# ostrosco/comms-rs

Hardware: NVIDIA B200
Metric: FIR/FFT Msamples/s (higher is better)
Workload: dtype f32

## Files before the change

comms-rs_b200/csrc/fir_tc_kernel.cu:

```cuda
#include <cuda_fp16.h>

#include <vector>

#include "fir_kernels.cuh"

namespace cb {

namespace tc {

constexpr int ROWS = 128;
constexpr int RS = 32;
constexpr int TILE = ROWS * RS;
constexpr int NCW = 6;
constexpr int NCONV = 32 * NCW;
constexpr int W_EPI = 2 * NCW;
constexpr int W_MMA = W_EPI + 4, W_TMA = W_EPI + 5;
constexpr int NTHREADS = 32 * (W_TMA + 1);
static_assert(W_EPI % 4 == 0, "epilogue warp w must own TMEM sub-partition w % 4");
constexpr int A_PART = 18432;
constexpr int A_STAGE = 2 * A_PART;
constexpr int OUT_PITCH = 272;
constexpr int OUT_WARP = 32 * OUT_PITCH;

struct Args {
    const float2 *x;
    const float2 *halo;
    float2 *y;
    const float2 *hist_in;
    float2 *hist_out;
    const uint4 *bimg;
    unsigned long long n;
    unsigned hist_len;
    float tap_inv_scale;
    unsigned *fix_count;
    unsigned *fix_list;
    const uint32_t *x16;
    uint32_t *y16;
    float in_scale, out_scale;
};

__device__ __forceinline__ int quant_i16(float v, float scale)
{
    const int q = __float2int_rz(__fmul_rn(scale, v));
    return min(max(q, -32768), 32767);
}
__device__ __forceinline__ uint32_t pack_i16(int lo, int hi) { return __byte_perm((uint32_t)lo, (uint32_t)hi, 0x5410); }
__device__ __forceinline__ float2 widen_iq16(uint32_t w, float scale)
{
    return make_float2(__fmul_rn(scale, (float)(int16_t)(w & 0xFFFFu)), __fmul_rn(scale, (float)(int16_t)(w >> 16)));
}

__device__ __forceinline__ void mbar_arrive(uint64_t *bar)
{
    asm volatile("mbarrier.arrive.shared::cta.b64 _, [%0];" ::"r"(smem_u32(bar)) : "memory");
}
__device__ __forceinline__ void tc_fence_before() { asm volatile("tcgen05.fence::before_thread_sync;" ::: "memory"); }
__device__ __forceinline__ void tc_fence_after() { asm volatile("tcgen05.fence::after_thread_sync;" ::: "memory"); }
__device__ __forceinline__ void tc_commit(uint64_t *bar)
{
    asm volatile("tcgen05.commit.cta_group::1.mbarrier::arrive::one.shared::cluster.b64 [%0];" ::"r"(smem_u32(bar))
                 : "memory");
}
__device__ __forceinline__ bool elect_one()
{
    uint32_t pred;
    asm volatile(
        "{\n"
        ".reg .pred P;\n"
        "elect.sync _|P, 0xffffffff;\n"
        "selp.u32 %0, 1, 0, P;\n"
        "}\n"
        : "=r"(pred));
    return pred != 0;
}
__device__ __forceinline__ void tc_mma(uint32_t tmem_d, uint64_t adesc, uint64_t bdesc, uint32_t idesc, uint32_t accumulate)
{
    asm volatile(
        "{\n"
        ".reg .pred p;\n"
        "setp.ne.b32 p, %4, 0;\n"
        "tcgen05.mma.cta_group::1.kind::f16 [%0], %1, %2, %3, p;\n"
        "}\n" ::"r"(tmem_d),
        "l"(adesc), "l"(bdesc), "r"(idesc), "r"(accumulate)
        : "memory");
}
__device__ __forceinline__ void tc_ld32(uint32_t taddr, uint32_t *r)
{
    asm volatile(
        "tcgen05.ld.sync.aligned.32x32b.x32.b32 "
        "{%0, %1, %2, %3, %4, %5, %6, %7, %8, %9, %10, %11, %12, %13, %14, %15, "
        "%16, %17, %18, %19, %20, %21, %22, %23, %24, %25, %26, %27, %28, %29, %30, %31}, [%32];\n"
        : "=r"(r[0]), "=r"(r[1]), "=r"(r[2]), "=r"(r[3]), "=r"(r[4]), "=r"(r[5]), "=r"(r[6]), "=r"(r[7]), "=r"(r[8]),
          "=r"(r[9]), "=r"(r[10]), "=r"(r[11]), "=r"(r[12]), "=r"(r[13]), "=r"(r[14]), "=r"(r[15]), "=r"(r[16]),
          "=r"(r[17]), "=r"(r[18]), "=r"(r[19]), "=r"(r[20]), "=r"(r[21]), "=r"(r[22]), "=r"(r[23]), "=r"(r[24]),
          "=r"(r[25]), "=r"(r[26]), "=r"(r[27]), "=r"(r[28]), "=r"(r[29]), "=r"(r[30]), "=r"(r[31])
        : "r"(taddr));
}
__device__ __forceinline__ void tc_wait_ld() { asm volatile("tcgen05.wait::ld.sync.aligned;" ::: "memory"); }

__device__ __forceinline__ uint64_t tc_desc(uint32_t saddr)
{
    uint64_t d = (uint64_t)((saddr >> 4) & 0x3FFF);
    d |= (uint64_t)1 << 16;
    d |= (uint64_t)(1024 >> 4) << 32;
    d |= (uint64_t)1 << 46;
    d |= (uint64_t)2 << 61;
    return d;
}

__device__ __forceinline__ uint32_t swz128(uint32_t o) { return o ^ (((o >> 7) & 7) << 4); }

__device__ __noinline__ float4 iq16_edge_pair(const Args &a, long long g, int halo);

#ifdef CB_FTC_STATS
__device__ unsigned long long *g_ftc_dbg = nullptr;
#define FTC_DECL unsigned long long st_[8] = {0}; long long t_ = clock64()
#define FTC_T(cond, k)                               \
    if (cond) {                                      \
        const long long now_ = clock64();            \
        st_[k] += (unsigned long long)(now_ - t_);   \
        t_ = now_;                                   \
    }
#define FTC_OUT(cond, role)                                                                            \
    if ((cond) && g_ftc_dbg != nullptr)                                                                \
        for (int k_ = 0; k_ < 8; ++k_) g_ftc_dbg[((size_t)blockIdx.x * 5 + (role)) * 8 + k_] = st_[k_]
#else
#define FTC_DECL
#define FTC_T(cond, k)
#define FTC_OUT(cond, role)
#endif

template <int KB, int NRAW, bool IQ16 = false, bool SMIN = false>
__global__ void __launch_bounds__(NTHREADS, 1) fir_tc_kernel(const __grid_constant__ Args a)
{
    constexpr int HALO = RS * (KB - 1);
    constexpr int NPAIR = (TILE + HALO) / 2;
    constexpr int NLD = (NPAIR + NCONV - 1) / NCONV;
    constexpr int B_BYTES = KB * 16384;
    constexpr uint32_t IDESC128 = (1u << 4) | ((128u >> 3) << 17) | ((128u >> 4) << 24);
    constexpr uint32_t IDESC64 = (1u << 4) | ((64u >> 3) << 17) | ((128u >> 4) << 24);

    extern __shared__ __align__(1024) unsigned char smem_raw[];
    unsigned char *smem = smem_raw + ((1024u - (smem_u32(smem_raw) & 1023u)) & 1023u);
    unsigned char *sB = smem;
    unsigned char *sA = smem + B_BYTES;
    unsigned char *sOut = sA + 2 * A_STAGE;
    constexpr int RAWB = (TILE + HALO) * (IQ16 ? 4 : 8);
    unsigned char *sRaw = sOut + 4 * OUT_WARP;
    __shared__ __align__(8) uint64_t raw_full[NRAW], raw_empty[NRAW];
    __shared__ __align__(8) uint64_t a_full[2], a_empty[2], t_full[2], t_empty[2], sc_ready[8];
    __shared__ uint32_t tmem_slot;
    __shared__ float red_max[2][2][NCW];
    __shared__ uint32_t red_min[2][2][NCW];
    __shared__ unsigned fix_seen[2];
    __shared__ float inv_scale[8];

    const int tid = threadIdx.x, warp = tid >> 5, lane = tid & 31;
    const unsigned long long ntiles = (a.n + TILE - 1) / TILE;

    if (tid == 0) {
        fix_seen[0] = fix_seen[1] = 0u;
        for (int i = 0; i < 2; ++i) {
            mbar_init(&a_full[i], NCONV);
            mbar_init(&a_empty[i], 1);
            mbar_init(&t_full[i], 1);
            mbar_init(&t_empty[i], 128);
        }
        for (int i = 0; i < 8; ++i) mbar_init(&sc_ready[i], 1);
        for (int i = 0; i < NRAW; ++i) {
            mbar_init(&raw_full[i], 1);
            mbar_init(&raw_empty[i], NCONV);
        }
        fence_mbar_init();
    }
    if (warp == W_MMA) {
        asm volatile("tcgen05.alloc.cta_group::1.sync.aligned.shared::cta.b32 [%0], %1;" ::"r"(smem_u32(&tmem_slot)),
                     "r"(256)
                     : "memory");
        asm volatile("tcgen05.relinquish_alloc_permit.cta_group::1.sync.aligned;" ::: "memory");
    }
    for (int i = tid; i < B_BYTES / 16; i += NTHREADS) reinterpret_cast<uint4 *>(sB)[i] = a.bimg[i];
    for (int i = tid; i < NRAW * RAWB / 16; i += NTHREADS) reinterpret_cast<uint4 *>(sRaw)[i] = make_uint4(0u, 0u, 0u, 0u);
    fence_proxy_async();
    tc_fence_before();
    __syncthreads();
    tc_fence_after();
    const uint32_t tmem_base = tmem_slot;

    if (warp == W_TMA) {
        unsigned long long it = 0;
        FTC_DECL;
        for (unsigned long long tile = blockIdx.x; tile < ntiles; tile += gridDim.x, ++it) {
            const int rs = (int)(it % NRAW);
            const uint32_t ph = (uint32_t)((it / NRAW) & 1);
            const long long g0 = (long long)tile * TILE - HALO;
            const long long g_lo = g0 < 0 ? 0 : g0;
            long long g_hi = g0 + TILE + HALO;
            if (g_hi > (long long)a.n) g_hi = (long long)a.n & (IQ16 ? ~3ll : ~1ll);
            if (g_hi < g_lo) g_hi = g_lo;
            FTC_T(lane == 0, 0);
            mbar_wait_long(&raw_empty[rs], ph ^ 1);
            FTC_T(lane == 0, 1);
            unsigned char *dstb = sRaw + rs * RAWB;
            if constexpr (IQ16) {
                if (lane == 0) mbar_arrive_expect_tx(&raw_full[rs], (uint32_t)((g_hi - g_lo) * 4));
                __syncwarp();
                for (long long g = g_lo + (long long)lane * 512; g < g_hi; g += 32 * 512) {
                    const long long n = g_hi - g < 512 ? g_hi - g : 512;
                    tma_load_1d(dstb + (g - g0) * 4, a.x16 + g, (uint32_t)(n * 4), &raw_full[rs]);
                }
                continue;
            }
            if (lane == 0) mbar_arrive_expect_tx(&raw_full[rs], (uint32_t)((g_hi - g_lo) * 8 + (g0 < 0 ? -g0 * 8 : 0)));
            __syncwarp();
            if (g0 < 0 && lane == 31) tma_load_1d(dstb, a.halo + (HALO + g0), (uint32_t)(-g0 * 8), &raw_full[rs]);
            for (long long g = g_lo + (long long)lane * 256; g < g_hi; g += 32 * 256) {
                const long long n = g_hi - g < 256 ? g_hi - g : 256;
                tma_load_1d(dstb + (g - g0) * 8, a.x + g, (uint32_t)(n * 8), &raw_full[rs]);
            }
        }
        FTC_OUT(lane == 0, 0);
    } else if (warp < W_EPI) {
        const int grp = warp / NCW, gt = tid - grp * NCONV, gw = warp - grp * NCW;
        if (a.hist_out != nullptr && blockIdx.x == 0 && grp == 0) {
            const long long H = a.hist_len;
            for (long long i = gt; i < H; i += NCONV) {
                const long long g = (long long)a.n - H + i;
                if constexpr (IQ16) a.hist_out[i] = g >= 0 ? widen_iq16(a.x16[g], a.in_scale) : a.hist_in[H + g];
                else a.hist_out[i] = g >= 0 ? a.x[g] : a.hist_in[H + g];
            }
        }
        unsigned long long it = grp;
        FTC_DECL;
        for (unsigned long long tile = blockIdx.x + (unsigned long long)grp * gridDim.x; tile < ntiles;
             tile += 2ull * gridDim.x, it += 2) {
            const int s = grp;
            const uint32_t ph = (uint32_t)((it >> 1) & 1);
            const long long t0 = (long long)tile * TILE;
            float4 raw[NLD];
            float mx = 0.f;
            uint32_t mnu = 0xffffffffu;
            const int rs = (int)(it % NRAW);
            FTC_T(gt == 0, 0);
            mbar_wait(&raw_full[rs], (uint32_t)((it / NRAW) & 1));
            FTC_T(gt == 0, 1);
            const float4 *rawt = reinterpret_cast<const float4 *>(sRaw + rs * RAWB);
            if constexpr (IQ16) {
                uint2 rw[NLD];
#pragma unroll
                for (int i = 0; i < NLD; ++i) {
                    const int q = gt + i * NCONV;
                    rw[i] = q < NPAIR ? reinterpret_cast<const uint2 *>(rawt)[q] : make_uint2(0u, 0u);
                }
#pragma unroll
                for (int i = 0; i < NLD; ++i) {
                    const float2 s0 = widen_iq16(rw[i].x, a.in_scale), s1 = widen_iq16(rw[i].y, a.in_scale);
                    raw[i] = make_float4(s0.x, s0.y, s1.x, s1.y);
                }
                if (t0 < HALO || t0 + TILE > ((long long)a.n & ~3ll)) {
#pragma unroll
                    for (int i = 0; i < NLD; ++i) {
                        const int q = gt + i * NCONV;
                        const long long g = t0 - HALO + 2 * q;
                        if (q < NPAIR && (g < 0 || g + 1 >= ((long long)a.n & ~3ll))) raw[i] = iq16_edge_pair(a, g, HALO);
                    }
                    if (t0 < HALO) {
#pragma unroll
                        for (int i = 0; i < NLD; ++i) {
                            const float4 v = raw[i];
                            mnu = min(mnu, quiet_key<SMIN>(v, fmaxf(fmaxf(fabsf(v.x), fabsf(v.y)), fmaxf(fabsf(v.z), fabsf(v.w)))));
                        }
                    }
                }
#pragma unroll
                for (int i = 0; i < NLD; ++i) {
                    const float4 v = raw[i];
                    mx = fmaxf(mx, fmaxf(fmaxf(fabsf(v.x), fabsf(v.y)), fmaxf(fabsf(v.z), fabsf(v.w))));
                }
            } else {
#pragma unroll
                for (int i = 0; i < NLD; ++i) {
                    const int q = gt + i * NCONV;
                    float4 v = make_float4(0.f, 0.f, 0.f, 0.f);
                    if (q < NPAIR) {
                        const long long g = t0 - HALO + 2 * q;
                        if (g < 0 || g + 1 < (long long)a.n) {
                            v = rawt[q];
                        } else if (g < (long long)a.n) {
                            const float2 t = a.x[g];
                            v = make_float4(t.x, t.y, 0.f, 0.f);
                        }
                    }
                    raw[i] = v;
                    const float pm = fmaxf(fmaxf(fabsf(v.x), fabsf(v.y)), fmaxf(fabsf(v.z), fabsf(v.w)));
                    mx = fmaxf(mx, pm);
                    mnu = min(mnu, quiet_key<SMIN>(v, pm));
                }
// ... 14 lines not shown
            mx = red_max[s][ph][0];
            mnu = red_min[s][ph][0];
#pragma unroll
            for (int w = 1; w < NCW; ++w) {
                mx = fmaxf(mx, red_max[s][ph][w]);
                mnu = min(mnu, red_min[s][ph][w]);
            }
            if (gt == 0 && a.fix_count != nullptr && mnu != 0xffffffffu && __uint_as_float(mnu + 1u) < mx * 9.5367431640625e-7f &&
                atomicExch(&fix_seen[s], (unsigned)tile + 1u) != (unsigned)tile + 1u)
                a.fix_list[atomicAdd(a.fix_count, 1u)] = (unsigned)tile;
            uint32_t eb = (__float_as_uint(mx) >> 23) & 0xFF;
            eb = (eb < 16 || eb == 255) ? 141 : eb;
            const float sc = __uint_as_float((268u - eb) << 23);
            if (gt == 0) {
                inv_scale[it & 7] = __uint_as_float((eb - 14u) << 23);
                mbar_arrive(&sc_ready[it & 7]);
            }

            FTC_T(gt == 0, 4);
            mbar_wait(&a_empty[s], ph ^ 1);
            FTC_T(gt == 0, 5);
            unsigned char *hi = sA + s * A_STAGE, *lo = hi + A_PART;
            __half2 nanacc = __floats2half2_rn(0.f, 0.f);
#pragma unroll
            for (int i = 0; i < NLD; ++i) {
                const int q = gt + i * NCONV;
                if (q < NPAIR) {
                    const float4 v = make_float4(raw[i].x * sc, raw[i].y * sc, raw[i].z * sc, raw[i].w * sc);
                    const __half2 h0 = __floats2half2_rn(v.x, v.y), h1 = __floats2half2_rn(v.z, v.w);
                    const float2 b0 = __half22float2(h0), b1 = __half22float2(h1);
                    const __half2 l0 = __floats2half2_rn(v.x - b0.x, v.y - b0.y);
                    const __half2 l1 = __floats2half2_rn(v.z - b1.x, v.w - b1.y);
                    nanacc = __hadd2(nanacc, __hadd2(l0, l1));
                    const uint32_t off = swz128((uint32_t)q * 8u);
                    uint2 ph2, pl2;
                    ph2.x = *reinterpret_cast<const uint32_t *>(&h0);
                    ph2.y = *reinterpret_cast<const uint32_t *>(&h1);
                    pl2.x = *reinterpret_cast<const uint32_t *>(&l0);
                    pl2.y = *reinterpret_cast<const uint32_t *>(&l1);
                    *reinterpret_cast<uint2 *>(hi + off) = ph2;
                    *reinterpret_cast<uint2 *>(lo + off) = pl2;
                }
            }
            fence_proxy_async();
            mbar_arrive(&a_full[s]);
            FTC_T(gt == 0, 6);
            if (a.fix_count != nullptr && (__hisnan(__low2half(nanacc)) || __hisnan(__high2half(nanacc))) &&
                atomicExch(&fix_seen[s], (unsigned)tile + 1u) != (unsigned)tile + 1u)
                a.fix_list[atomicAdd(a.fix_count, 1u)] = (unsigned)tile;
        }
        FTC_OUT(gt == 0, 1 + grp);
    } else if (warp == W_MMA) {
        unsigned long long it = 0;
        const uint64_t bd0 = tc_desc(smem_u32(sB)), ad0 = tc_desc(smem_u32(sA));
        FTC_DECL;
        for (unsigned long long tile = blockIdx.x; tile < ntiles; tile += gridDim.x, ++it) {
            const int s = (int)(it & 1);
            const uint32_t ph = (uint32_t)((it >> 1) & 1);
            FTC_T(lane == 0, 0);
            mbar_wait_long(&t_empty[s], ph ^ 1);
            FTC_T(lane == 0, 1);
            mbar_wait_long(&a_full[s], ph);
            FTC_T(lane == 0, 2);
            tc_fence_after();
            const uint64_t ahi = ad0 + (uint64_t)((s * A_STAGE) >> 4), alo = ahi + (uint64_t)(A_PART >> 4);
            const uint32_t d = tmem_base + (uint32_t)s * 128u;
            if (elect_one()) {
#pragma unroll
                for (int t = 0; t < KB * 4; ++t) {
                    const uint64_t aoff = (uint64_t)(((t >> 2) * 128 + (t & 3) * 32) >> 4);
                    const uint64_t boff = (uint64_t)(((t >> 2) * 16384 + (t & 3) * 32) >> 4);
                    tc_mma(d, ahi + aoff, bd0 + boff, IDESC128, t > 0 ? 1u : 0u);
                    tc_mma(d, alo + aoff, bd0 + boff, IDESC64, 1u);
                }
                tc_commit(&a_empty[s]);
                tc_commit(&t_full[s]);
            }
            __syncwarp();
        }
        FTC_OUT(lane == 0, 3);
    } else {
        const int e = warp - W_EPI;
        unsigned char *stage = sOut + e * OUT_WARP;
        const bool direct = IQ16 ? (reinterpret_cast<uintptr_t>(a.y16) & 31) == 0 : (reinterpret_cast<uintptr_t>(a.y) & 31) == 0;
        unsigned long long it = 0;
        FTC_DECL;
        for (unsigned long long tile = blockIdx.x; tile < ntiles; tile += gridDim.x, ++it) {
            const int s = (int)(it & 1);
            const uint32_t ph = (uint32_t)((it >> 1) & 1);
            const long long t0 = (long long)tile * TILE;
            FTC_T(e == 0 && lane == 0, 0);
            mbar_wait(&sc_ready[it & 7], (uint32_t)((it >> 3) & 1));
            const float k0 = inv_scale[it & 7], k1 = a.tap_inv_scale;
            mbar_wait_long(&t_full[s], ph);
            FTC_T(e == 0 && lane == 0, 1);
            tc_fence_after();
            const uint32_t taddr = tmem_base + ((uint32_t)(32 * e) << 16) + (uint32_t)s * 128u;
            const long long row = t0 + (long long)(32 * e + lane) * RS;
            if constexpr (IQ16) {
#pragma unroll
                for (int half = 0; half < 2; ++half) {
                    uint32_t p[32], r[32];
                    tc_ld32(taddr + half * 32, p);
                    tc_ld32(taddr + 64 + half * 32, r);
                    tc_wait_ld();
#pragma unroll
                    for (int c = 0; c < 2; ++c) {
                        float w[8];
#pragma unroll
                        for (int u = 0; u < 8; ++u) {
                            const float vr = (__uint_as_float(p[16 * c + 2 * u]) + __uint_as_float(r[16 * c + 2 * u])) * k0 * k1;
                            const float vi = (__uint_as_float(p[16 * c + 2 * u + 1]) + __uint_as_float(r[16 * c + 2 * u + 1])) * k0 * k1;
                            w[u] = __uint_as_float(pack_i16(quant_i16(vr, a.out_scale), quant_i16(vi, a.out_scale)));
                        }
                        const long long sidx = row + 16 * half + 8 * c;
                        if (direct && sidx + 7 < (long long)a.n) {
                            stg_stream8(reinterpret_cast<float *>(a.y16 + sidx), w);
                        } else {
#pragma unroll
                            for (int u = 0; u < 8; ++u)
                                if (sidx + u < (long long)a.n) a.y16[sidx + u] = __float_as_uint(w[u]);
                        }
                    }
                }
                tc_fence_before();
                mbar_arrive(&t_empty[s]);
                FTC_T(e == 0 && lane == 0, 2);
                continue;
            }
            if (direct) {
#pragma unroll
                for (int half = 0; half < 2; ++half) {
                    uint32_t p[32], r[32];
                    tc_ld32(taddr + half * 32, p);
                    tc_ld32(taddr + 64 + half * 32, r);
                    tc_wait_ld();
#pragma unroll
                    for (int c = 0; c < 4; ++c) {
                        float v[8];
#pragma unroll
                        for (int u = 0; u < 8; ++u)
                            v[u] = (__uint_as_float(p[8 * c + u]) + __uint_as_float(r[8 * c + u])) * k0 * k1;
                        const long long sidx = row + 16 * half + 4 * c;
                        if (sidx + 3 < (long long)a.n) {
                            stg_stream8(reinterpret_cast<float *>(a.y + sidx), v);
                        } else {
#pragma unroll
                            for (int u = 0; u < 4; ++u)
                                if (sidx + u < (long long)a.n) a.y[sidx + u] = make_float2(v[2 * u], v[2 * u + 1]);
                        }
                    }
                }
                tc_fence_before();
                mbar_arrive(&t_empty[s]);
                FTC_T(e == 0 && lane == 0, 2);
                continue;
            }
#pragma unroll
            for (int half = 0; half < 2; ++half) {
                uint32_t p[32], r[32];
                tc_ld32(taddr + half * 32, p);
                tc_ld32(taddr + 64 + half * 32, r);
                tc_wait_ld();
#pragma unroll
                for (int c = 0; c < 8; ++c) {
                    float4 v;
                    v.x = (__uint_as_float(p[4 * c]) + __uint_as_float(r[4 * c])) * k0 * k1;
                    v.y = (__uint_as_float(p[4 * c + 1]) + __uint_as_float(r[4 * c + 1])) * k0 * k1;
                    v.z = (__uint_as_float(p[4 * c + 2]) + __uint_as_float(r[4 * c + 2])) * k0 * k1;
                    v.w = (__uint_as_float(p[4 * c + 3]) + __uint_as_float(r[4 * c + 3])) * k0 * k1;
                    *reinterpret_cast<float4 *>(stage + lane * OUT_PITCH + half * 128 + c * 16) = v;
                }
            }
            tc_fence_before();
            mbar_arrive(&t_empty[s]);
            __syncwarp();
            const long long row0 = t0 + (long long)(32 * e) * RS;
#pragma unroll 4
            for (int i = 0; i < 16; ++i) {
                const int idx = i * 32 + lane, rr = idx >> 4, c = idx & 15;
                const float4 v = *reinterpret_cast<const float4 *>(stage + rr * OUT_PITCH + c * 16);
                const long long sidx = row0 + (long long)rr * RS + 2 * c;
                if (sidx + 1 < (long long)a.n) stg_stream(reinterpret_cast<float4 *>(a.y + sidx), v);
                else if (sidx < (long long)a.n) a.y[sidx] = make_float2(v.x, v.y);
            }
            __syncwarp();
            FTC_T(e == 0 && lane == 0, 2);
        }
        FTC_OUT(e == 0 && lane == 0, 4);
    }

    tc_fence_before();
    __syncthreads();
    if (warp == W_MMA) {
        asm volatile("tcgen05.dealloc.cta_group::1.sync.aligned.b32 %0, %1;" ::"r"(tmem_base), "r"(256) : "memory");
    }
}

__device__ __noinline__ float4 iq16_edge_pair(const Args &a, long long g, int halo)
{
    float2 s0 = make_float2(0.f, 0.f), s1 = s0;
    if (g < 0) {
        s0 = a.halo[halo + g];
        s1 = a.halo[halo + g + 1];
    } else {
        if (g < (long long)a.n) s0 = widen_iq16(a.x16[g], a.in_scale);
        if (g + 1 < (long long)a.n) s1 = widen_iq16(a.x16[g + 1], a.in_scale);
    }
    return make_float4(s0.x, s0.y, s1.x, s1.y);
}

}

size_t fir_tc_image_bytes(uint32_t ntaps)
{
    const int kb = 1 + (int)ceil_div(ntaps ? ntaps : 1, (size_t)tc::RS);
    return (size_t)kb * 16384;
}

int fir_tc_kblocks(uint32_t ntaps) { return 1 + (int)ceil_div(ntaps ? ntaps : 1, (size_t)tc::RS); }

void fir_tc_build_image(const float2 *taps, uint32_t ntaps, unsigned char *img, float *tap_inv_scale)
{
    const int KB = fir_tc_kblocks(ntaps);
    const int HALO = tc::RS * (KB - 1);
    float mx = 0.f;
    for (uint32_t k = 0; k < ntaps; ++k) mx = fmaxf(mx, fmaxf(fabsf(taps[k].x), fabsf(taps[k].y)));
    uint32_t bits;
    memcpy(&bits, &mx, 4);
    uint32_t eb = (bits >> 23) & 0xFF;
    if (eb < 16 || eb == 255) eb = 141;
    const uint32_t sb = (268u - eb) << 23, ib = (eb - 14u) << 23;
    float sc;
    memcpy(&sc, &sb, 4);
    memcpy(tap_inv_scale, &ib, 4);
    memset(img, 0, (size_t)KB * 16384);
    for (int n = 0; n < 64; ++n) {
        const int i = n >> 1, c = n & 1;
        for (int k = 0; k < 64 * KB; ++k) {
            const int j = k >> 1, d = k & 1;
            const int t = i + HALO - j;
            float v = 0.f;
            if (t >= 0 && t < (int)ntaps) {
                const float hr = taps[t].x, hi = taps[t].y;
                v = c == 0 ? (d == 0 ? hr : -hi) : (d == 0 ? hi : hr);
            }
            v *= sc;
            const __half h = __float2half_rn(v);
            const __half l = __float2half_rn(v - __half2float(h));
            const int kb = k >> 6, kk = k & 63;
            uint32_t o_hi = (uint32_t)n * 128u + (uint32_t)kk * 2u;
            uint32_t o_lo = (uint32_t)(64 + n) * 128u + (uint32_t)kk * 2u;
            o_hi ^= ((o_hi >> 7) & 7) << 4;
            o_lo ^= ((o_lo >> 7) & 7) << 4;
            memcpy(img + (size_t)kb * 16384 + o_hi, &h, 2);
            memcpy(img + (size_t)kb * 16384 + o_lo, &l, 2);
        }
    }
}

template <int KB, bool IQ16, bool SMIN>
static int launch_tc_kb(const tc::Args &a, cudaStream_t stream)
{
    constexpr int RAWB = (tc::TILE + tc::RS * (KB - 1)) * (IQ16 ? 4 : 8);
    constexpr int BASE = KB * 16384 + 2 * tc::A_STAGE + 4 * tc::OUT_WARP + 1024;
    constexpr int NRAW = BASE + 2 * RAWB <= 227 * 1024 ? 2 : 1;
    constexpr int SMEM = BASE + NRAW * RAWB;
    static_assert(SMEM <= 227 * 1024, "fir_tc: shared memory budget");
    auto kern = tc::fir_tc_kernel<KB, NRAW, IQ16, SMIN>;
    CB_CUDA(cudaFuncSetAttribute(kern, cudaFuncAttributeMaxDynamicSharedMemorySize, SMEM));
    const unsigned long long ntiles = (a.n + tc::TILE - 1) / tc::TILE;
    int dev = 0, sms = 148;
    cudaGetDevice(&dev);
    cudaDeviceGetAttribute(&sms, cudaDevAttrMultiProcessorCount, dev);
    const unsigned grid = (unsigned)(ntiles < (unsigned long long)sms ? ntiles : (unsigned long long)sms);
    kern<<<grid, tc::NTHREADS, SMEM, stream>>>(a);
    count_launch();
    CB_CUDA(cudaGetLastError());
    return CB_OK;
}

bool fir_tc_applicable(const FirSeg &seg)
{
    if (seg.interp != 1 || seg.decim != 1 || seg.ntaps == 0 || seg.ntaps > 128) return false;
    const int KB = fir_tc_kblocks(seg.ntaps);
    const uint32_t halo = (uint32_t)tc::RS * (KB - 1);
    if (seg.hist_len < halo) return false;
    const float2 *h = seg.hist_in + (seg.hist_len - halo);
    return ((reinterpret_cast<uintptr_t>(seg.x) | reinterpret_cast<uintptr_t>(seg.y) | reinterpret_cast<uintptr_t>(h)) & 15) == 0;
}

bool fir_tc_iq16_applicable(const FirSeg &seg, const int16_t *x16, const int16_t *y16)
{
    if (seg.interp != 1 || seg.decim != 1 || seg.ntaps == 0 || seg.ntaps > 128) return false;
    const int KB = fir_tc_kblocks(seg.ntaps);
    const uint32_t halo = (uint32_t)tc::RS * (KB - 1);
    if (seg.hist_len < halo) return false;
    return (reinterpret_cast<uintptr_t>(x16) & 15) == 0 && (reinterpret_cast<uintptr_t>(y16) & 3) == 0;
}

static int launch_tc(const FirSeg &seg, tc::Args &a, bool iq16, const FirTcPlan &plan, const float2 *taps_dev,
                     cudaStream_t stream)
{
    if (seg.n_in == 0) return CB_OK;
    const int KB = fir_tc_kblocks(seg.ntaps);
    a.halo = seg.hist_in + (seg.hist_len - (uint32_t)tc::RS * (KB - 1));
    a.hist_in = seg.hist_in;
    a.hist_out = seg.hist_out;
    a.bimg = reinterpret_cast<const uint4 *>(plan.bimg_dev);
    a.n = seg.n_in;
    a.hist_len = seg.hist_len;
    a.tap_inv_scale = plan.tap_inv_scale;
    FirFix *fix = plan.fix;
    const bool fixup = fix != nullptr && fix->dev != nullptr && taps_dev != nullptr &&
                       fix->cap >= ceil_div(seg.n_in, (size_t)tc::TILE);
    a.fix_count = fixup ? fix->dev + (fix->calls & 1u) : nullptr;
    a.fix_list = fixup ? fix->dev + 2 : nullptr;
    const int sel = KB * 4 + (iq16 ? 2 : 0) + (plan.sample_min ? 1 : 0);
    int rc;
    switch (sel) {
#define CB_TC_CASE(kb)                                                          \
// ... 40 lines not shown
```

comms-rs_b200/csrc/common.cuh:

```cuda
#pragma once

#include <cuda_runtime.h>
#include <stdint.h>
#include <stdio.h>
#include <string>

#include "../../include/comms_b200.h"

namespace cb {

void set_error(const char *fmt, ...);
int cuda_fail(cudaError_t e, const char *what, const char *file, int line);
int current_device();
void count_launch();

#define CB_CUDA(call)                                                        \
    do {                                                                     \
        cudaError_t e__ = (call);                                            \
        if (e__ != cudaSuccess) return cb::cuda_fail(e__, #call, __FILE__, __LINE__); \
    } while (0)

#define CB_REQUIRE(cond, status, ...)                                        \
    do {                                                                     \
        if (!(cond)) {                                                       \
// ... 84 lines not shown
    asm volatile(
        "cp.async.bulk.shared::cluster.global.mbarrier::complete_tx::bytes.L2::cache_hint [%0], [%1], %2, [%3], %4;" ::"r"(
            smem_u32(dst_smem)),
        "l"(src_gmem), "r"(bytes), "r"(smem_u32(bar)), "l"(pol)
        : "memory");
}

__device__ __forceinline__ void tma_store_1d(void *dst_gmem, const void *src_smem, uint32_t bytes)
{
    asm volatile("cp.async.bulk.global.shared::cta.bulk_group [%0], [%1], %2;" ::"l"(dst_gmem),
                 "r"(smem_u32(src_smem)), "r"(bytes)
                 : "memory");
}
__device__ __forceinline__ void tma_store_commit() { asm volatile("cp.async.bulk.commit_group;" ::: "memory"); }
__device__ __forceinline__ void tma_store_wait_all() { asm volatile("cp.async.bulk.wait_group 0;" ::: "memory"); }
__device__ __forceinline__ void tma_store_wait_read() { asm volatile("cp.async.bulk.wait_group.read 0;" ::: "memory"); }

__device__ __forceinline__ float4 ldg_stream(const float4 *p)
{
    float4 v;
    asm volatile("ld.global.nc.L1::no_allocate.v4.f32 {%0,%1,%2,%3}, [%4];"
                 : "=f"(v.x), "=f"(v.y), "=f"(v.z), "=f"(v.w)
                 : "l"(p));
    return v;
}
__device__ __forceinline__ void ldg_stream8(const float *p, float *v)
{
    asm volatile("ld.global.nc.L1::no_allocate.v8.f32 {%0,%1,%2,%3,%4,%5,%6,%7}, [%8];"
                 : "=f"(v[0]), "=f"(v[1]), "=f"(v[2]), "=f"(v[3]), "=f"(v[4]), "=f"(v[5]), "=f"(v[6]), "=f"(v[7])
                 : "l"(p));
}
__device__ __forceinline__ float2 ldg_stream2(const float2 *p)
{
    float2 v;
    asm volatile("ld.global.nc.L1::no_allocate.v2.f32 {%0,%1}, [%2];" : "=f"(v.x), "=f"(v.y) : "l"(p));
    return v;
}
__device__ __forceinline__ void stg_stream(float4 *p, float4 v)
{
    asm volatile("st.global.L1::no_allocate.v4.f32 [%0], {%1,%2,%3,%4};" ::"l"(p), "f"(v.x), "f"(v.y), "f"(v.z),
                 "f"(v.w)
                 : "memory");
}
__device__ __forceinline__ void stg_stream8(float *p, const float *v)
{
    asm volatile("st.global.L1::no_allocate.v8.f32 [%0], {%1,%2,%3,%4,%5,%6,%7,%8};" ::"l"(p), "f"(v[0]), "f"(v[1]), "f"(v[2]),
                 "f"(v[3]), "f"(v[4]), "f"(v[5]), "f"(v[6]), "f"(v[7])
                 : "memory");
}
__device__ __forceinline__ void stg_stream2(float2 *p, float2 v)
{
    asm volatile("st.global.L1::no_allocate.v2.f32 [%0], {%1,%2};" ::"l"(p), "f"(v.x), "f"(v.y) : "memory");
}
#endif

}
```

Measured before the change: 334,400.

## Drop epilogue smem staging, guarantee double-buffered raw input, add L2 prefetch

Removes the 4-warp output staging buffer in shared memory. The unaligned-output path now writes two float4 streaming stores straight from TMEM registers instead of bouncing through smem. The freed shared memory lets two raw-input stages always fit, and a static assert now requires NRAW >= 2. The TMA producer issues a bulk L2 prefetch for the tile it will load next in that slot, and uses a doubled set of full-barriers indexed modulo 2*NRAW. This aims to hide global-load latency, at the cost of more complex barrier-phase logic and less coalesced direct stores in the unaligned case.

```diff
diff --git a/comms-rs_b200/csrc/fir_tc_kernel.cu b/comms-rs_b200/csrc/fir_tc_kernel.cu
--- a/comms-rs_b200/csrc/fir_tc_kernel.cu
+++ b/comms-rs_b200/csrc/fir_tc_kernel.cu
@@ -1,5 +1,6 @@
 #include <cuda_fp16.h>
 
+#include <type_traits>
 #include <vector>
 
 #include "fir_kernels.cuh"
@@ -19,8 +20,6 @@
 static_assert(W_EPI % 4 == 0, "epilogue warp w must own TMEM sub-partition w % 4");
 constexpr int A_PART = 18432;
 constexpr int A_STAGE = 2 * A_PART;
-constexpr int OUT_PITCH = 272;
-constexpr int OUT_WARP = 32 * OUT_PITCH;
 
 struct Args {
     const float2 *x;
@@ -124,10 +123,19 @@
 #define FTC_OUT(cond, role)                                                                            \
     if ((cond) && g_ftc_dbg != nullptr)                                                                \
         for (int k_ = 0; k_ < 8; ++k_) g_ftc_dbg[((size_t)blockIdx.x * 5 + (role)) * 8 + k_] = st_[k_]
+__device__ unsigned long long *g_ftc_clk = nullptr;
+#define FTC_CLK(slot)                                                                                  \
+    if (threadIdx.x == 0 && g_ftc_clk != nullptr) {                                                    \
+        unsigned long long ns_;                                                                        \
+        asm volatile("mov.u64 %0, %%globaltimer;" : "=l"(ns_));                                        \
+        g_ftc_clk[blockIdx.x * 4 + 2 * (slot)] = ns_;                                                  \
+        g_ftc_clk[blockIdx.x * 4 + 2 * (slot) + 1] = (unsigned long long)clock64();                    \
+    }
 #else
 #define FTC_DECL
 #define FTC_T(cond, k)
 #define FTC_OUT(cond, role)
+#define FTC_CLK(slot)
 #endif
 
 template <int KB, int NRAW, bool IQ16 = false, bool SMIN = false>
@@ -144,10 +152,9 @@
     unsigned char *smem = smem_raw + ((1024u - (smem_u32(smem_raw) & 1023u)) & 1023u);
     unsigned char *sB = smem;
     unsigned char *sA = smem + B_BYTES;
-    unsigned char *sOut = sA + 2 * A_STAGE;
     constexpr int RAWB = (TILE + HALO) * (IQ16 ? 4 : 8);
-    unsigned char *sRaw = sOut + 4 * OUT_WARP;
-    __shared__ __align__(8) uint64_t raw_full[NRAW], raw_empty[NRAW];
+    unsigned char *sRaw = sA + 2 * A_STAGE;
+    __shared__ __align__(8) uint64_t raw_full[2 * NRAW], raw_empty[NRAW];
     __shared__ __align__(8) uint64_t a_full[2], a_empty[2], t_full[2], t_empty[2], sc_ready[8];
     __shared__ uint32_t tmem_slot;
     __shared__ float red_max[2][2][NCW];
@@ -155,6 +162,7 @@
     __shared__ unsigned fix_seen[2];
     __shared__ float inv_scale[8];
 
+    FTC_CLK(0);
     const int tid = threadIdx.x, warp = tid >> 5, lane = tid & 31;
     const unsigned long long ntiles = (a.n + TILE - 1) / TILE;
 
@@ -167,10 +175,8 @@
             mbar_init(&t_empty[i], 128);
         }
         for (int i = 0; i < 8; ++i) mbar_init(&sc_ready[i], 1);
-        for (int i = 0; i < NRAW; ++i) {
-            mbar_init(&raw_full[i], 1);
-            mbar_init(&raw_empty[i], NCONV);
-        }
+        for (int i = 0; i < 2 * NRAW; ++i) mbar_init(&raw_full[i], 1);
+        for (int i = 0; i < NRAW; ++i) mbar_init(&raw_empty[i], NCONV);
         fence_mbar_init();
     }
     if (warp == W_MMA) {
@@ -188,11 +194,23 @@
     const uint32_t tmem_base = tmem_slot;
 
     if (warp == W_TMA) {
+        auto prefetch_next = [&](unsigned long long tile) {
+            const unsigned long long nt = tile + (unsigned long long)NRAW * gridDim.x;
+            if (nt >= ntiles) return;
+            const long long lo = (long long)nt * TILE - HALO;
+            long long hi = lo + TILE + HALO;
+            if (hi > (long long)a.n) hi = (long long)a.n & (IQ16 ? ~3ll : ~1ll);
+            if (hi > lo)
+                asm volatile("cp.async.bulk.prefetch.L2.global [%0], %1;" ::"l"(IQ16 ? (const void *)(a.x16 + lo) : (const void *)(a.x + lo)),
+                             "r"((uint32_t)((hi - lo) * (IQ16 ? 4 : 8)))
+                             : "memory");
+        };
         unsigned long long it = 0;
         FTC_DECL;
         for (unsigned long long tile = blockIdx.x; tile < ntiles; tile += gridDim.x, ++it) {
             const int rs = (int)(it % NRAW);
             const uint32_t ph = (uint32_t)((it / NRAW) & 1);
+            uint64_t *full = &raw_full[it % (2 * NRAW)];
             const long long g0 = (long long)tile * TILE - HALO;
             const long long g_lo = g0 < 0 ? 0 : g0;
             long long g_hi = g0 + TILE + HALO;
@@ -203,21 +221,23 @@
             FTC_T(lane == 0, 1);
             unsigned char *dstb = sRaw + rs * RAWB;
             if constexpr (IQ16) {
-                if (lane == 0) mbar_arrive_expect_tx(&raw_full[rs], (uint32_t)((g_hi - g_lo) * 4));
+                if (lane == 0) mbar_arrive_expect_tx(full, (uint32_t)((g_hi - g_lo) * 4));
                 __syncwarp();
                 for (long long g = g_lo + (long long)lane * 512; g < g_hi; g += 32 * 512) {
                     const long long n = g_hi - g < 512 ? g_hi - g : 512;
-                    tma_load_1d(dstb + (g - g0) * 4, a.x16 + g, (uint32_t)(n * 4), &raw_full[rs]);
-                }
+                    tma_load_1d(dstb + (g - g0) * 4, a.x16 + g, (uint32_t)(n * 4), full);
+                }
+                if (lane == 0) prefetch_next(tile);
                 continue;
             }
-            if (lane == 0) mbar_arrive_expect_tx(&raw_full[rs], (uint32_t)((g_hi - g_lo) * 8 + (g0 < 0 ? -g0 * 8 : 0)));
+            if (lane == 0) mbar_arrive_expect_tx(full, (uint32_t)((g_hi - g_lo) * 8 + (g0 < 0 ? -g0 * 8 : 0)));
             __syncwarp();
-            if (g0 < 0 && lane == 31) tma_load_1d(dstb, a.halo + (HALO + g0), (uint32_t)(-g0 * 8), &raw_full[rs]);
+            if (g0 < 0 && lane == 31) tma_load_1d(dstb, a.halo + (HALO + g0), (uint32_t)(-g0 * 8), full);
             for (long long g = g_lo + (long long)lane * 256; g < g_hi; g += 32 * 256) {
                 const long long n = g_hi - g < 256 ? g_hi - g : 256;
-                tma_load_1d(dstb + (g - g0) * 8, a.x + g, (uint32_t)(n * 8), &raw_full[rs]);
-            }
+                tma_load_1d(dstb + (g - g0) * 8, a.x + g, (uint32_t)(n * 8), full);
+            }
+            if (lane == 0) prefetch_next(tile);
         }
         FTC_OUT(lane == 0, 0);
     } else if (warp < W_EPI) {
@@ -242,7 +262,7 @@
             uint32_t mnu = 0xffffffffu;
             const int rs = (int)(it % NRAW);
             FTC_T(gt == 0, 0);
-            mbar_wait(&raw_full[rs], (uint32_t)((it / NRAW) & 1));
+            mbar_wait(&raw_full[it % (2 * NRAW)], (uint32_t)((it / (2 * NRAW)) & 1));
             FTC_T(gt == 0, 1);
             const float4 *rawt = reinterpret_cast<const float4 *>(sRaw + rs * RAWB);
             if constexpr (IQ16) {
@@ -392,7 +412,6 @@
         FTC_OUT(lane == 0, 3);
     } else {
         const int e = warp - W_EPI;
-        unsigned char *stage = sOut + e * OUT_WARP;
         const bool direct = IQ16 ? (reinterpret_cast<uintptr_t>(a.y16) & 31) == 0 : (reinterpret_cast<uintptr_t>(a.y) & 31) == 0;
         unsigned long long it = 0;
         FTC_DECL;
@@ -439,7 +458,7 @@
                 FTC_T(e == 0 && lane == 0, 2);
                 continue;
             }
-            if (direct) {
+            auto drain = [&](auto wide) {
 #pragma unroll
                 for (int half = 0; half < 2; ++half) {
                     uint32_t p[32], r[32];
@@ -454,7 +473,12 @@
                             v[u] = (__uint_as_float(p[8 * c + u]) + __uint_as_float(r[8 * c + u])) * k0 * k1;
                         const long long sidx = row + 16 * half + 4 * c;
                         if (sidx + 3 < (long long)a.n) {
-                            stg_stream8(reinterpret_cast<float *>(a.y + sidx), v);
+                            if constexpr (decltype(wide)::value) {
+                                stg_stream8(reinterpret_cast<float *>(a.y + sidx), v);
+                            } else {
+                                stg_stream(reinterpret_cast<float4 *>(a.y + sidx), make_float4(v[0], v[1], v[2], v[3]));
+                                stg_stream(reinterpret_cast<float4 *>(a.y + sidx + 2), make_float4(v[4], v[5], v[6], v[7]));
+                            }
                         } else {
 #pragma unroll
                             for (int u = 0; u < 4; ++u)
@@ -462,40 +486,11 @@
                         }
                     }
                 }
-                tc_fence_before();
-                mbar_arrive(&t_empty[s]);
-                FTC_T(e == 0 && lane == 0, 2);
-                continue;
-            }
-#pragma unroll
-            for (int half = 0; half < 2; ++half) {
-                uint32_t p[32], r[32];
-                tc_ld32(taddr + half * 32, p);
-                tc_ld32(taddr + 64 + half * 32, r);
-                tc_wait_ld();
-#pragma unroll
-                for (int c = 0; c < 8; ++c) {
-                    float4 v;
-                    v.x = (__uint_as_float(p[4 * c]) + __uint_as_float(r[4 * c])) * k0 * k1;
-                    v.y = (__uint_as_float(p[4 * c + 1]) + __uint_as_float(r[4 * c + 1])) * k0 * k1;
-                    v.z = (__uint_as_float(p[4 * c + 2]) + __uint_as_float(r[4 * c + 2])) * k0 * k1;
-                    v.w = (__uint_as_float(p[4 * c + 3]) + __uint_as_float(r[4 * c + 3])) * k0 * k1;
-                    *reinterpret_cast<float4 *>(stage + lane * OUT_PITCH + half * 128 + c * 16) = v;
-                }
-            }
+            };
+            if (direct) drain(std::true_type{});
+            else drain(std::false_type{});
             tc_fence_before();
             mbar_arrive(&t_empty[s]);
-            __syncwarp();
-            const long long row0 = t0 + (long long)(32 * e) * RS;
-#pragma unroll 4
-            for (int i = 0; i < 16; ++i) {
-                const int idx = i * 32 + lane, rr = idx >> 4, c = idx & 15;
-                const float4 v = *reinterpret_cast<const float4 *>(stage + rr * OUT_PITCH + c * 16);
-                const long long sidx = row0 + (long long)rr * RS + 2 * c;
-                if (sidx + 1 < (long long)a.n) stg_stream(reinterpret_cast<float4 *>(a.y + sidx), v);
-                else if (sidx < (long long)a.n) a.y[sidx] = make_float2(v.x, v.y);
-            }
-            __syncwarp();
             FTC_T(e == 0 && lane == 0, 2);
         }
         FTC_OUT(e == 0 && lane == 0, 4);
@@ -503,6 +498,7 @@
 
     tc_fence_before();
     __syncthreads();
+    FTC_CLK(1);
     if (warp == W_MMA) {
         asm volatile("tcgen05.dealloc.cta_group::1.sync.aligned.b32 %0, %1;" ::"r"(tmem_base), "r"(256) : "memory");
     }
@@ -574,10 +570,12 @@
 static int launch_tc_kb(const tc::Args &a, cudaStream_t stream)
 {
     constexpr int RAWB = (tc::TILE + tc::RS * (KB - 1)) * (IQ16 ? 4 : 8);
-    constexpr int BASE = KB * 16384 + 2 * tc::A_STAGE + 4 * tc::OUT_WARP + 1024;
-    constexpr int NRAW = BASE + 2 * RAWB <= 227 * 1024 ? 2 : 1;
+    constexpr int BASE = KB * 16384 + 2 * tc::A_STAGE + 1024;
+    constexpr int BUDGET = 227 * 1024 - 1024;
+    constexpr int FIT = (BUDGET - BASE) / RAWB;
+    constexpr int NRAW = FIT < 2 ? FIT : 2;
     constexpr int SMEM = BASE + NRAW * RAWB;
-    static_assert(SMEM <= 227 * 1024, "fir_tc: shared memory budget");
+    static_assert(NRAW >= 2 && SMEM <= BUDGET, "fir_tc: shared memory budget");
     auto kern = tc::fir_tc_kernel<KB, NRAW, IQ16, SMIN>;
     CB_CUDA(cudaFuncSetAttribute(kern, cudaFuncAttributeMaxDynamicSharedMemorySize, SMEM));
     const unsigned long long ntiles = (a.n + tc::TILE - 1) / tc::TILE;
```

Result: slower. 322,200 (median of 6 runs) (-3.7%).

## Move FIR tap matrix into tensor memory and store epilogue directly from TMEM

Applied to the files above, without the earlier changes.

Moves the tap matrix from shared memory into tensor memory and issues MMAs with A taken from TMEM. The input tile is now the B operand, so the instruction descriptors swap M and N and the host tap image is re-laid out. The output staging buffers in shared memory are removed. The epilogue reads accumulators with 16x256b loads and writes scalar streaming stores straight to global, with a lane shuffle for the IQ16 packing. This frees shared memory for raw input buffering and drops the staging round trip, but allocates all 512 TMEM columns and replaces vector stores with many 4-byte stores.

```diff
diff --git a/comms-rs_b200/csrc/common.cuh b/comms-rs_b200/csrc/common.cuh
--- a/comms-rs_b200/csrc/common.cuh
+++ b/comms-rs_b200/csrc/common.cuh
@@ -160,6 +160,10 @@
 {
     asm volatile("st.global.L1::no_allocate.v2.f32 [%0], {%1,%2};" ::"l"(p), "f"(v.x), "f"(v.y) : "memory");
 }
+__device__ __forceinline__ void stg_stream1(float *p, float v)
+{
+    asm volatile("st.global.L1::no_allocate.f32 [%0], %1;" ::"l"(p), "f"(v) : "memory");
+}
 #endif
 
 }
diff --git a/comms-rs_b200/csrc/fir_tc_kernel.cu b/comms-rs_b200/csrc/fir_tc_kernel.cu
--- a/comms-rs_b200/csrc/fir_tc_kernel.cu
+++ b/comms-rs_b200/csrc/fir_tc_kernel.cu
@@ -1,5 +1,6 @@
 #include <cuda_fp16.h>
 
+#include <type_traits>
 #include <vector>
 
 #include "fir_kernels.cuh"
@@ -19,8 +20,8 @@
 static_assert(W_EPI % 4 == 0, "epilogue warp w must own TMEM sub-partition w % 4");
 constexpr int A_PART = 18432;
 constexpr int A_STAGE = 2 * A_PART;
-constexpr int OUT_PITCH = 272;
-constexpr int OUT_WARP = 32 * OUT_PITCH;
+constexpr uint32_t TM_TAPS = 256;
+constexpr uint32_t TM_COLS = 512;
 
 struct Args {
     const float2 *x;
@@ -73,21 +74,21 @@
         : "=r"(pred));
     return pred != 0;
 }
-__device__ __forceinline__ void tc_mma(uint32_t tmem_d, uint64_t adesc, uint64_t bdesc, uint32_t idesc, uint32_t accumulate)
+__device__ __forceinline__ void tc_mma_ts(uint32_t tmem_d, uint32_t tmem_a, uint64_t bdesc, uint32_t idesc, uint32_t accumulate)
 {
     asm volatile(
         "{\n"
         ".reg .pred p;\n"
         "setp.ne.b32 p, %4, 0;\n"
-        "tcgen05.mma.cta_group::1.kind::f16 [%0], %1, %2, %3, p;\n"
+        "tcgen05.mma.cta_group::1.kind::f16 [%0], [%1], %2, %3, p;\n"
         "}\n" ::"r"(tmem_d),
-        "l"(adesc), "l"(bdesc), "r"(idesc), "r"(accumulate)
+        "r"(tmem_a), "l"(bdesc), "r"(idesc), "r"(accumulate)
         : "memory");
 }
-__device__ __forceinline__ void tc_ld32(uint32_t taddr, uint32_t *r)
+__device__ __forceinline__ void tc_ld16x64(uint32_t taddr, uint32_t *r)
 {
     asm volatile(
-        "tcgen05.ld.sync.aligned.32x32b.x32.b32 "
+        "tcgen05.ld.sync.aligned.16x256b.x8.b32 "
         "{%0, %1, %2, %3, %4, %5, %6, %7, %8, %9, %10, %11, %12, %13, %14, %15, "
         "%16, %17, %18, %19, %20, %21, %22, %23, %24, %25, %26, %27, %28, %29, %30, %31}, [%32];\n"
         : "=r"(r[0]), "=r"(r[1]), "=r"(r[2]), "=r"(r[3]), "=r"(r[4]), "=r"(r[5]), "=r"(r[6]), "=r"(r[7]), "=r"(r[8]),
@@ -96,7 +97,28 @@
           "=r"(r[25]), "=r"(r[26]), "=r"(r[27]), "=r"(r[28]), "=r"(r[29]), "=r"(r[30]), "=r"(r[31])
         : "r"(taddr));
 }
+__device__ __forceinline__ void tc_ld16x32(uint32_t taddr, uint32_t *r)
+{
+    asm volatile(
+        "tcgen05.ld.sync.aligned.16x256b.x4.b32 "
+        "{%0, %1, %2, %3, %4, %5, %6, %7, %8, %9, %10, %11, %12, %13, %14, %15}, [%16];\n"
+        : "=r"(r[0]), "=r"(r[1]), "=r"(r[2]), "=r"(r[3]), "=r"(r[4]), "=r"(r[5]), "=r"(r[6]), "=r"(r[7]), "=r"(r[8]),
+          "=r"(r[9]), "=r"(r[10]), "=r"(r[11]), "=r"(r[12]), "=r"(r[13]), "=r"(r[14]), "=r"(r[15])
+        : "r"(taddr));
+}
 __device__ __forceinline__ void tc_wait_ld() { asm volatile("tcgen05.wait::ld.sync.aligned;" ::: "memory"); }
+__device__ __forceinline__ void tc_st32(uint32_t taddr, const uint32_t *r)
+{
+    asm volatile(
+        "tcgen05.st.sync.aligned.32x32b.x32.b32 [%0], "
+        "{%1, %2, %3, %4, %5, %6, %7, %8, %9, %10, %11, %12, %13, %14, %15, %16, "
+        "%17, %18, %19, %20, %21, %22, %23, %24, %25, %26, %27, %28, %29, %30, %31, %32};\n" ::"r"(taddr),
+        "r"(r[0]), "r"(r[1]), "r"(r[2]), "r"(r[3]), "r"(r[4]), "r"(r[5]), "r"(r[6]), "r"(r[7]), "r"(r[8]), "r"(r[9]),
+        "r"(r[10]), "r"(r[11]), "r"(r[12]), "r"(r[13]), "r"(r[14]), "r"(r[15]), "r"(r[16]), "r"(r[17]), "r"(r[18]),
+        "r"(r[19]), "r"(r[20]), "r"(r[21]), "r"(r[22]), "r"(r[23]), "r"(r[24]), "r"(r[25]), "r"(r[26]), "r"(r[27]),
+        "r"(r[28]), "r"(r[29]), "r"(r[30]), "r"(r[31])
+        : "memory");
+}
 
 __device__ __forceinline__ uint64_t tc_desc(uint32_t saddr)
 {
@@ -136,17 +158,15 @@
     constexpr int HALO = RS * (KB - 1);
     constexpr int NPAIR = (TILE + HALO) / 2;
     constexpr int NLD = (NPAIR + NCONV - 1) / NCONV;
-    constexpr int B_BYTES = KB * 16384;
+    static_assert(TM_TAPS + 32 * KB <= TM_COLS, "fir_tc: tap matrix and accumulators exceed tensor memory");
     constexpr uint32_t IDESC128 = (1u << 4) | ((128u >> 3) << 17) | ((128u >> 4) << 24);
-    constexpr uint32_t IDESC64 = (1u << 4) | ((64u >> 3) << 17) | ((128u >> 4) << 24);
+    constexpr uint32_t IDESC64 = (1u << 4) | ((128u >> 3) << 17) | ((64u >> 4) << 24);
 
     extern __shared__ __align__(1024) unsigned char smem_raw[];
     unsigned char *smem = smem_raw + ((1024u - (smem_u32(smem_raw) & 1023u)) & 1023u);
-    unsigned char *sB = smem;
-    unsigned char *sA = smem + B_BYTES;
-    unsigned char *sOut = sA + 2 * A_STAGE;
+    unsigned char *sA = smem;
     constexpr int RAWB = (TILE + HALO) * (IQ16 ? 4 : 8);
-    unsigned char *sRaw = sOut + 4 * OUT_WARP;
+    unsigned char *sRaw = sA + 2 * A_STAGE;
     __shared__ __align__(8) uint64_t raw_full[NRAW], raw_empty[NRAW];
     __shared__ __align__(8) uint64_t a_full[2], a_empty[2], t_full[2], t_empty[2], sc_ready[8];
     __shared__ uint32_t tmem_slot;
@@ -175,17 +195,36 @@
     }
     if (warp == W_MMA) {
         asm volatile("tcgen05.alloc.cta_group::1.sync.aligned.shared::cta.b32 [%0], %1;" ::"r"(smem_u32(&tmem_slot)),
-                     "r"(256)
+                     "r"(TM_COLS)
                      : "memory");
         asm volatile("tcgen05.relinquish_alloc_permit.cta_group::1.sync.aligned;" ::: "memory");
     }
-    for (int i = tid; i < B_BYTES / 16; i += NTHREADS) reinterpret_cast<uint4 *>(sB)[i] = a.bimg[i];
     for (int i = tid; i < NRAW * RAWB / 16; i += NTHREADS) reinterpret_cast<uint4 *>(sRaw)[i] = make_uint4(0u, 0u, 0u, 0u);
     fence_proxy_async();
     tc_fence_before();
     __syncthreads();
     tc_fence_after();
     const uint32_t tmem_base = tmem_slot;
+    if (warp >= W_EPI && warp < W_MMA) {
+        const int row = 32 * (warp - W_EPI) + lane;
+        const uint4 *src = a.bimg + (size_t)row * (KB * 8);
+        for (int c = 0; c < KB; ++c) {
+            uint32_t v[32];
+#pragma unroll
+            for (int q = 0; q < 8; ++q) {
+                const uint4 w = src[8 * c + q];
+                v[4 * q] = w.x;
+                v[4 * q + 1] = w.y;
+                v[4 * q + 2] = w.z;
+                v[4 * q + 3] = w.w;
+            }
+            tc_st32(tmem_base + ((uint32_t)(32 * (warp - W_EPI)) << 16) + TM_TAPS + 32u * c, v);
+        }
+        asm volatile("tcgen05.wait::st.sync.aligned;" ::: "memory");
+    }
+    tc_fence_before();
+    __syncthreads();
+    tc_fence_after();
 
     if (warp == W_TMA) {
         unsigned long long it = 0;
@@ -363,7 +402,8 @@
         FTC_OUT(gt == 0, 1 + grp);
     } else if (warp == W_MMA) {
         unsigned long long it = 0;
-        const uint64_t bd0 = tc_desc(smem_u32(sB)), ad0 = tc_desc(smem_u32(sA));
+        const uint64_t bd0 = tc_desc(smem_u32(sA));
+        const uint32_t taps = tmem_base + TM_TAPS;
         FTC_DECL;
         for (unsigned long long tile = blockIdx.x; tile < ntiles; tile += gridDim.x, ++it) {
             const int s = (int)(it & 1);
@@ -374,15 +414,14 @@
             mbar_wait_long(&a_full[s], ph);
             FTC_T(lane == 0, 2);
             tc_fence_after();
-            const uint64_t ahi = ad0 + (uint64_t)((s * A_STAGE) >> 4), alo = ahi + (uint64_t)(A_PART >> 4);
+            const uint64_t bhi = bd0 + (uint64_t)((s * A_STAGE) >> 4), blo = bhi + (uint64_t)(A_PART >> 4);
             const uint32_t d = tmem_base + (uint32_t)s * 128u;
             if (elect_one()) {
 #pragma unroll
                 for (int t = 0; t < KB * 4; ++t) {
-                    const uint64_t aoff = (uint64_t)(((t >> 2) * 128 + (t & 3) * 32) >> 4);
-                    const uint64_t boff = (uint64_t)(((t >> 2) * 16384 + (t & 3) * 32) >> 4);
-                    tc_mma(d, ahi + aoff, bd0 + boff, IDESC128, t > 0 ? 1u : 0u);
-                    tc_mma(d, alo + aoff, bd0 + boff, IDESC64, 1u);
+                    const uint64_t boff = (uint64_t)(((t >> 2) * 128 + (t & 3) * 32) >> 4);
+                    tc_mma_ts(d, taps + 8u * t, bhi + boff, IDESC128, t > 0 ? 1u : 0u);
+                    tc_mma_ts(d, taps + 8u * t, blo + boff, IDESC64, 1u);
                 }
                 tc_commit(&a_empty[s]);
                 tc_commit(&t_full[s]);
@@ -392,8 +431,7 @@
         FTC_OUT(lane == 0, 3);
     } else {
         const int e = warp - W_EPI;
-        unsigned char *stage = sOut + e * OUT_WARP;
-        const bool direct = IQ16 ? (reinterpret_cast<uintptr_t>(a.y16) & 31) == 0 : (reinterpret_cast<uintptr_t>(a.y) & 31) == 0;
+        const int q = lane & 3, c = (lane >> 2) & 1, i0 = 8 * e + (lane >> 3);
         unsigned long long it = 0;
         FTC_DECL;
         for (unsigned long long tile = blockIdx.x; tile < ntiles; tile += gridDim.x, ++it) {
@@ -407,95 +445,51 @@
             FTC_T(e == 0 && lane == 0, 1);
             tc_fence_after();
             const uint32_t taddr = tmem_base + ((uint32_t)(32 * e) << 16) + (uint32_t)s * 128u;
-            const long long row = t0 + (long long)(32 * e + lane) * RS;
-            if constexpr (IQ16) {
-#pragma unroll
-                for (int half = 0; half < 2; ++half) {
-                    uint32_t p[32], r[32];
-                    tc_ld32(taddr + half * 32, p);
-                    tc_ld32(taddr + 64 + half * 32, r);
+            const long long o0 = t0 + i0 + 32 * (2 * q + (IQ16 ? c : 0));
+            const long long rem = (long long)a.n - o0;
+            constexpr int NCH = IQ16 ? 4 : 2, NJ = 16 / NCH;
+            auto drain = [&](auto checked) {
+#pragma unroll
+                for (int half = 0; half < NCH; ++half) {
+                    uint32_t r[2][4 * NJ];
+                    if constexpr (NJ == 8) {
+                        tc_ld16x64(taddr + 64u * half, r[0]);
+                        tc_ld16x64(taddr + (16u << 16) + 64u * half, r[1]);
+                    } else {
+                        tc_ld16x32(taddr + 32u * half, r[0]);
+                        tc_ld16x32(taddr + (16u << 16) + 32u * half, r[1]);
+                    }
                     tc_wait_ld();
 #pragma unroll
-                    for (int c = 0; c < 2; ++c) {
-                        float w[8];
-#pragma unroll
-                        for (int u = 0; u < 8; ++u) {
-                            const float vr = (__uint_as_float(p[16 * c + 2 * u]) + __uint_as_float(r[16 * c + 2 * u])) * k0 * k1;
-                            const float vi = (__uint_as_float(p[16 * c + 2 * u + 1]) + __uint_as_float(r[16 * c + 2 * u + 1])) * k0 * k1;
-                            w[u] = __uint_as_float(pack_i16(quant_i16(vr, a.out_scale), quant_i16(vi, a.out_scale)));
-                        }
-                        const long long sidx = row + 16 * half + 8 * c;
-                        if (direct && sidx + 7 < (long long)a.n) {
-                            stg_stream8(reinterpret_cast<float *>(a.y16 + sidx), w);
-                        } else {
-#pragma unroll
-                            for (int u = 0; u < 8; ++u)
-                                if (sidx + u < (long long)a.n) a.y16[sidx + u] = __float_as_uint(w[u]);
+                    for (int b = 0; b < 2; ++b) {
+#pragma unroll
+                        for (int j = 0; j < NJ; ++j) {
+                            float v[2];
+#pragma unroll
+                            for (int u = 0; u < 2; ++u)
+                                v[u] = (__uint_as_float(r[0][4 * j + 2 * b + u]) + __uint_as_float(r[1][4 * j + 2 * b + u])) * k0 * k1;
+                            const int k = 4 * b + 32 * (8 * NJ * half + 8 * j);
+                            if constexpr (IQ16) {
+                                const float send = c ? v[0] : v[1];
+                                const float recv = __shfl_xor_sync(0xffffffffu, send, 4);
+                                const float vr = c ? recv : v[0], vi = c ? v[1] : recv;
+                                const uint32_t w = pack_i16(quant_i16(vr, a.out_scale), quant_i16(vi, a.out_scale));
+                                if (!decltype(checked)::value || k < rem)
+                                    stg_stream1(reinterpret_cast<float *>(a.y16 + o0 + k), __uint_as_float(w));
+                            } else {
+#pragma unroll
+                                for (int u = 0; u < 2; ++u)
+                                    if (!decltype(checked)::value || k + 32 * u < rem)
+                                        stg_stream1(reinterpret_cast<float *>(a.y + o0 + k + 32 * u) + c, v[u]);
+                            }
                         }
                     }
                 }
-                tc_fence_before();
-                mbar_arrive(&t_empty[s]);
-                FTC_T(e == 0 && lane == 0, 2);
-                continue;
-            }
-            if (direct) {
-#pragma unroll
-                for (int half = 0; half < 2; ++half) {
-                    uint32_t p[32], r[32];
-                    tc_ld32(taddr + half * 32, p);
-                    tc_ld32(taddr + 64 + half * 32, r);
-                    tc_wait_ld();
-#pragma unroll
-                    for (int c = 0; c < 4; ++c) {
-                        float v[8];
-#pragma unroll
-                        for (int u = 0; u < 8; ++u)
-                            v[u] = (__uint_as_float(p[8 * c + u]) + __uint_as_float(r[8 * c + u])) * k0 * k1;
-                        const long long sidx = row + 16 * half + 4 * c;
-                        if (sidx + 3 < (long long)a.n) {
-                            stg_stream8(reinterpret_cast<float *>(a.y + sidx), v);
-                        } else {
-#pragma unroll
-                            for (int u = 0; u < 4; ++u)
-                                if (sidx + u < (long long)a.n) a.y[sidx + u] = make_float2(v[2 * u], v[2 * u + 1]);
-                        }
-                    }
-                }
-                tc_fence_before();
-                mbar_arrive(&t_empty[s]);
-                FTC_T(e == 0 && lane == 0, 2);
-                continue;
-            }
-#pragma unroll
-            for (int half = 0; half < 2; ++half) {
-                uint32_t p[32], r[32];
-                tc_ld32(taddr + half * 32, p);
-                tc_ld32(taddr + 64 + half * 32, r);
-                tc_wait_ld();
-#pragma unroll
-                for (int c = 0; c < 8; ++c) {
-                    float4 v;
-                    v.x = (__uint_as_float(p[4 * c]) + __uint_as_float(r[4 * c])) * k0 * k1;
-                    v.y = (__uint_as_float(p[4 * c + 1]) + __uint_as_float(r[4 * c + 1])) * k0 * k1;
-                    v.z = (__uint_as_float(p[4 * c + 2]) + __uint_as_float(r[4 * c + 2])) * k0 * k1;
-                    v.w = (__uint_as_float(p[4 * c + 3]) + __uint_as_float(r[4 * c + 3])) * k0 * k1;
-                    *reinterpret_cast<float4 *>(stage + lane * OUT_PITCH + half * 128 + c * 16) = v;
-                }
-            }
+            };
+            if (t0 + TILE <= (long long)a.n) drain(std::false_type());
+            else drain(std::true_type());
             tc_fence_before();
             mbar_arrive(&t_empty[s]);
-            __syncwarp();
-            const long long row0 = t0 + (long long)(32 * e) * RS;
-#pragma unroll 4
-            for (int i = 0; i < 16; ++i) {
-                const int idx = i * 32 + lane, rr = idx >> 4, c = idx & 15;
-                const float4 v = *reinterpret_cast<const float4 *>(stage + rr * OUT_PITCH + c * 16);
-                const long long sidx = row0 + (long long)rr * RS + 2 * c;
-                if (sidx + 1 < (long long)a.n) stg_stream(reinterpret_cast<float4 *>(a.y + sidx), v);
-                else if (sidx < (long long)a.n) a.y[sidx] = make_float2(v.x, v.y);
-            }
-            __syncwarp();
             FTC_T(e == 0 && lane == 0, 2);
         }
         FTC_OUT(e == 0 && lane == 0, 4);
@@ -504,7 +498,7 @@
     tc_fence_before();
     __syncthreads();
     if (warp == W_MMA) {
-        asm volatile("tcgen05.dealloc.cta_group::1.sync.aligned.b32 %0, %1;" ::"r"(tmem_base), "r"(256) : "memory");
+        asm volatile("tcgen05.dealloc.cta_group::1.sync.aligned.b32 %0, %1;" ::"r"(tmem_base), "r"(TM_COLS) : "memory");
     }
 }
 
@@ -559,13 +553,9 @@
             v *= sc;
             const __half h = __float2half_rn(v);
             const __half l = __float2half_rn(v - __half2float(h));
-            const int kb = k >> 6, kk = k & 63;
-            uint32_t o_hi = (uint32_t)n * 128u + (uint32_t)kk * 2u;
-            uint32_t o_lo = (uint32_t)(64 + n) * 128u + (uint32_t)kk * 2u;
-            o_hi ^= ((o_hi >> 7) & 7) << 4;
-            o_lo ^= ((o_lo >> 7) & 7) << 4;
-            memcpy(img + (size_t)kb * 16384 + o_hi, &h, 2);
-            memcpy(img + (size_t)kb * 16384 + o_lo, &l, 2);
+            const size_t row = (size_t)(32 * (n >> 4) + (n & 15));
+            memcpy(img + row * 128 * KB + 2 * k, &h, 2);
+            memcpy(img + (row + 16) * 128 * KB + 2 * k, &l, 2);
         }
     }
 }
@@ -574,7 +564,7 @@
 static int launch_tc_kb(const tc::Args &a, cudaStream_t stream)
 {
     constexpr int RAWB = (tc::TILE + tc::RS * (KB - 1)) * (IQ16 ? 4 : 8);
-    constexpr int BASE = KB * 16384 + 2 * tc::A_STAGE + 4 * tc::OUT_WARP + 1024;
+    constexpr int BASE = 2 * tc::A_STAGE + 1024;
     constexpr int NRAW = BASE + 2 * RAWB <= 227 * 1024 ? 2 : 1;
     constexpr int SMEM = BASE + NRAW * RAWB;
     static_assert(SMEM <= 227 * 1024, "fir_tc: shared memory budget");
```

After: 350,000 before, 340,600 after, median of 6. 0.973x the previous value.
